# mitenjain/nanopore

Measured on AMD Instinct MI355X. Metric: DP cells/sec (banded pair-HMM realign: forward + backward + posterior per cell), higher is better.
Workload: dtype f32

## Files before the change

### include/nprealign.h

```cpp
#ifndef NPREALIGN_H
#define NPREALIGN_H

#include <stddef.h>
#include <stdint.h>

#ifdef __cplusplus
extern "C" {
#endif

#define NPR_ABI_VERSION 1

#define NPR_OK 0
#define NPR_ERR_INVALID (-1)
#define NPR_ERR_ZERO_PROB (-2)
#define NPR_ERR_CAPACITY (-3)
#define NPR_ERR_MODEL (-4)
#define NPR_ERR_NO_DEVICE (-5)
#define NPR_ERR_HIP (-6)
#define NPR_ERR_BAND_TOO_WIDE (-7)
#define NPR_ERR_NOMEM (-8)
#define NPR_ERR_STATE (-9)

#define NPR_OP_M 0
#define NPR_OP_I 1
// ... 57 lines not shown
#define NPR_OPT_RELEASE_SCRATCH 2
#define NPR_OPT_KERNEL 3
#define NPR_OPT_ARITH 4
#define NPR_OPT_PAIR 5
#define NPR_OPT_NO_TILE 6
#define NPR_OPT_NO_WIDE 7
#define NPR_OPT_TILE_RS 8
#define NPR_OPT_TILE_WAVES 9
#define NPR_OPT_HOST_MEA 13
#define NPR_OPT_MEA_RING_ONLY 14
#define NPR_OPT_MEA_GLOBAL_SORT 15
#define NPR_OPT_EM_GENERIC 17
#define NPR_OPT_MEA_WIDE_OPS 20
#define NPR_OPT_EM_TILE 21
#define NPR_OPT_FINISH_TEXT 22
#define NPR_OPT_COUNT 23
int32_t npr_ctx_option(npr_ctx *ctx, int32_t option, int64_t value);

int32_t npr_set_hmm(npr_ctx *ctx, int32_t slot, const double *T25, const double *E80);

int32_t npr_batch_create(npr_ctx *ctx, const npr_params *params, int64_t n_reads, int64_t n_refs,
                         const uint8_t *ref, const int64_t *ref_off, const int32_t *ref_index,
                         const uint8_t *read, const int64_t *read_off, const int32_t *guide_ops,
                         const int64_t *guide_off, const int32_t *model_slot, npr_batch **out);
int32_t npr_batch_create_at(npr_ctx *ctx, const npr_params *params, int64_t n_reads, int64_t n_refs,
                            const uint8_t *ref, const int64_t *ref_off, const int32_t *ref_index,
                            const uint8_t *read, const int64_t *read_off, const int32_t *guide_ops,
                            const int64_t *guide_off, const int64_t *guide_start, const int32_t *model_slot,
                            npr_batch **out);
int32_t npr_batch_run(npr_batch *b, float *kernel_ms);
int32_t npr_batch_finish(npr_batch *b);
void npr_batch_destroy(npr_batch *b);

int32_t npr_batch_get_stats(const npr_batch *b, npr_batch_stats *st);
int32_t npr_batch_class_stats(const npr_batch *b, int64_t *tasks, int64_t *cells, int32_t cap);
int32_t npr_batch_segment_arith(const npr_batch *b, int64_t *seg_off, int32_t *arith, int64_t cap);
int32_t npr_batch_results(const npr_batch *b, npr_read_result *out );
int32_t npr_batch_ops(const npr_batch *b, int64_t *ops_off, int32_t *ops, int64_t cap_pairs);
int32_t npr_batch_ops_packed(const npr_batch *b, int64_t *ops_off, uint32_t *words, int64_t cap_words);
int32_t npr_batch_pairs(const npr_batch *b, int64_t *pair_off, int32_t *x, int32_t *y, float *p, int64_t cap);
int32_t npr_batch_debug_set_pairs(npr_batch *b, int64_t read, const int32_t *x, const int32_t *y, const float *p, int64_t n, int32_t task_status);

#define NPR_STATS_WORDS 40
int32_t npr_batch_align_stats(npr_batch *b, int32_t *stats );
int32_t npr_align_stats(npr_ctx *ctx, int64_t n_reads, int64_t n_refs, const uint8_t *ref, const int64_t *ref_off,
                        const int32_t *ref_index, const uint8_t *read, const int64_t *read_off, const int32_t *ops,
                        const int64_t *ops_off, const int64_t *start, int32_t *stats );


int32_t npr_kmer_counts(npr_ctx *ctx, int32_t k, int64_t n_seqs, const uint8_t *seq, const int64_t *seq_off,
                        int64_t *counts );
int32_t npr_kmer_counts_groups(npr_ctx *ctx, int32_t k, int64_t n_seqs, const uint8_t *text, const int64_t *seq_begin,
                               const int64_t *seq_end, const int32_t *group, int32_t n_groups,
                               int64_t *counts );
int32_t npr_align_indel_kmers(npr_ctx *ctx, int32_t k, int64_t n_reads, int64_t n_refs, const uint8_t *ref, const int64_t *ref_off,
                              const int32_t *ref_index, const uint8_t *read, const int64_t *read_off, const int32_t *ops,
// ... 92 lines not shown
```

### nanopore_amd/_lib.py

```python
import ctypes as C
import os

import numpy as np

_HERE = os.path.dirname(os.path.abspath(__file__))
LIB_LOADED = False


def want_hw_queues(n=8):
    have = os.environ.get("GPU_MAX_HW_QUEUES")
    if have is None:
        os.environ["GPU_MAX_HW_QUEUES"] = str(n)
    if os.environ.get("NPR_TIMING") or os.environ.get("NPR_JOB_TRACE"):
        import sys
        sys.stderr.write("[npr] GPU_MAX_HW_QUEUES %s%s\n" % (
            "left at the host's %s" % have if have is not None else "set to %d for this process and its children" % n,
            " (the library is already loaded: the runtime may have read it before)" if LIB_LOADED and have is None else ""))


LIB_PATH = os.environ.get("NPR_LIB") or os.path.join(_HERE, "libnprealign.so")

OK = 0
ERR_INVALID, ERR_ZERO_PROB, ERR_CAPACITY, ERR_MODEL, ERR_NO_DEVICE, ERR_HIP, ERR_BAND_TOO_WIDE, ERR_NOMEM, \
    ERR_STATE = -1, -2, -3, -4, -5, -6, -7, -8, -9
OP_M, OP_I, OP_D = 0, 1, 2
BAND_ANCHOR, BAND_FIXED = 0, 1
MODE_REALIGN, MODE_RESCORE_ORIGINAL, MODE_ALL_POSTERIORS, MODE_EXPECTATIONS = 0, 1, 2, 3
OPT_OVERLAP = 1
OPT_RELEASE_SCRATCH = 2
OPTIONS = dict(kernel=3, arith=4, pair=5, no_tile=6, no_wide=7, tile_rs=8, tile_waves=9, host_mea=13, mea_ring_only=14,
               mea_global_sort=15, em_generic=17, mea_wide_ops=20, em_tile=21, finish_text=22)
OPT_FINISH_TEXT = 22
KERNEL_GENERIC, ARITH_CELL, PAIR_NEVER, PAIR_LONG, PAIR_ALL = 1, 1, 1, 2, 3
STATS_WORDS = 40
KMER_MAX_K = 6
KMER_MAX_GROUPS = 64
SAM_COLS = 16
PILEUP_WORDS = 8
MAX_MODELS = 8
E_DEAD = -(1 << 28)


class Params(C.Structure):
    _fields_ = [
        ("band_mode", C.c_int32),
        ("diagonal_expansion", C.c_int32),
# ... 39 lines not shown
    ]


class NprError(RuntimeError):
    def __init__(self, code, where, detail=""):
        self.code = code
        msg = "%s failed: %s (%d)" % (where, strerror(code), code)
        if detail:
            msg += " -- " + detail
        RuntimeError.__init__(self, msg)


EXPORTS = [
    "npr_abi_version", "npr_strerror", "npr_create", "npr_destroy", "npr_last_error", "npr_set_hmm",
    "npr_batch_create", "npr_batch_create_at", "npr_batch_run", "npr_batch_finish", "npr_batch_destroy", "npr_batch_get_stats", "npr_batch_class_stats",
    "npr_batch_results", "npr_batch_ops", "npr_batch_ops_packed", "npr_batch_pairs", "npr_batch_debug_set_pairs", "npr_batch_dense", "npr_batch_rs_forward", "npr_batch_expectations",
    "npr_batch_align_stats", "npr_align_stats", "npr_batch_plan_check", "npr_batch_base_expectations",
    "npr_kmer_counts", "npr_kmer_counts_groups", "npr_align_indel_kmers", "npr_batch_indel_kmers",
    "npr_pileup_create", "npr_pileup_destroy", "npr_pileup_add_batch", "npr_pileup_add", "npr_pileup_counts", "npr_pileup_depth",
    "npr_realign_batch",
    "npr_plan_create", "npr_plan_destroy", "npr_plan_segments", "npr_plan_segment_info",
    "npr_plan_segment_band", "npr_plan_frame_schedule", "npr_plan_stripes", "npr_format_cigars", "npr_format_cigars_packed", "npr_format_sam_records", "npr_chain_hits", "npr_mea_cigar", "npr_rescore", "npr_encode_bases",
    "npr_sam_index", "npr_sam_parse", "npr_sam_guides", "npr_sam_splice", "npr_fasta_index", "npr_fasta_pack", "npr_fastq_index", "npr_names_mark",
    "npr_batch_create_spans", "npr_chain_merge", "npr_ctx_option", "npr_batch_segment_arith",
    "npr_cigar_text_packed", "npr_batch_cigar_text", "npr_sam_splice_text",
]

_lib = None


def load():
# ... 36 lines not shown
    L.npr_batch_finish.argtypes = [vp]
    L.npr_batch_destroy.restype = None
    L.npr_batch_destroy.argtypes = [vp]
    L.npr_batch_get_stats.restype = i32
    L.npr_batch_get_stats.argtypes = [vp, C.POINTER(BatchStats)]
    L.npr_batch_results.restype = i32
    L.npr_batch_results.argtypes = [vp, vp]
    L.npr_batch_ops.restype = i32
    L.npr_batch_ops.argtypes = [vp, vp, vp, i64]
    L.npr_batch_ops_packed.restype = i32
    L.npr_batch_ops_packed.argtypes = [vp, vp, vp, i64]
    L.npr_batch_pairs.restype = i32
    L.npr_batch_pairs.argtypes = [vp, vp, vp, vp, vp, i64]
    L.npr_batch_debug_set_pairs.restype = i32
    L.npr_batch_debug_set_pairs.argtypes = [vp, i64, vp, vp, vp, i64, i32]
    L.npr_batch_expectations.restype = i32
    L.npr_batch_expectations.argtypes = [vp, vp, vp, vp, C.POINTER(C.c_float)]
    L.npr_batch_base_expectations.restype = i32
    L.npr_batch_base_expectations.argtypes = [vp, vp, i64, vp, vp, vp]
    L.npr_batch_plan_check.restype = i64
    L.npr_batch_plan_check.argtypes = [vp, vp]
    L.npr_batch_align_stats.restype = i32
    L.npr_batch_align_stats.argtypes = [vp, vp]
    L.npr_align_stats.restype = i32
    L.npr_align_stats.argtypes = [vp, i64, i64, vp, vp, vp, vp, vp, vp, vp, vp, vp]
    L.npr_kmer_counts.restype = i32
    L.npr_kmer_counts.argtypes = [vp, i32, i64, vp, vp, vp]
    L.npr_kmer_counts_groups.restype = i32
    L.npr_kmer_counts_groups.argtypes = [vp, i32, i64, vp, vp, vp, vp, i32, vp]
    L.npr_align_indel_kmers.restype = i32
# ... 84 lines not shown
```

### nanopore_amd/csrc/npr_api_internal.h

```cpp
#pragma once
#include <hip/hip_runtime.h>

#include <algorithm>
#include <atomic>
#include <chrono>
#include <cmath>
#include <cstdio>
#include <cstdlib>
#include <cstring>
#include <exception>
#include <memory>
#include <mutex>
#include <new>
#include <numeric>
#include <string>
#include <thread>
#include <type_traits>
#include <vector>

#include "npr_device.h"
#include "npr_internal.h"
#include "npr_sched.h"
#include "npr_threads.h"

// ... 246 lines not shown
    int64_t packed_cap = 0;
    bool have_pairs_form = false, have_packed_form = false;
    bool ops_from_guide = false;
    bool rs_staged = false;
    int rs_shift = 0;
    std::vector<int64_t> rs_columns, rs_kept;
    DevBuf<int32_t> d_rs_gy;
    DevBuf<int64_t> d_rs_gx_off;
    std::vector<int64_t> pair_off;
    std::vector<Pair> pairs;
    bool pairs_ready = false;
    std::vector<int64_t> task_dst;
    const uint32_t *dev_ops = nullptr;
    const int64_t *dev_od = nullptr;
    uint64_t dev_ops_epoch = 0;
    std::unique_ptr<char[]> text;
    int64_t text_cap = 0;
    std::vector<int64_t> text_off;
    bool text_ready = false, words_on_device = false;
};

struct npr_pileup {
    npr_ctx *ctx = nullptr;
    std::vector<int64_t> len;
    std::vector<int64_t> base;
    int64_t rows = 0;
    DevBuf<int32_t> tab;
    DevBuf<int32_t> diff;
    DevBuf<int32_t> tile;
    DevBuf<int64_t> dbase;
// ... 99 lines not shown
```

### nanopore_amd/csrc/npr_device.h

```cpp
#pragma once
#include <cstdint>

#include "npr_internal.h"
#include "npr_band.h"

namespace npr {

struct Task {
    int64_t x_off;
    int64_t y_off;
    int64_t band_off;
    int64_t pair_off;
    int32_t lX, lY;
    int32_t D;
    int32_t pair_cap;
    int32_t flags;
    int32_t model;
    int32_t xs, ys;
    int32_t read;
    int32_t cells_pad;
    int64_t ctl_off;
    int64_t tile_off;
    int64_t rowmask_off;
};
// ... 68 lines not shown
int launch_stair(const KernelArgs &a, int R, int grid, void *stream);
int launch_wide(const KernelArgs &a, int R, int NW, int grid, void *stream);
int launch_em_stair(const KernelArgs &a, int R, int grid, void *stream);
size_t em_stair_lds_bytes();
struct MeaArgs {
    const Task *tasks;
    const TaskOut *outs;
    int32_t ntasks, n_reads;
    const int32_t *px, *py;
    const float *pp;
    const int64_t *rx_off;
    const int64_t *ry_off;
    const int64_t *rp_off;
    int32_t *cnt, *start, *colsum;
    int32_t *sx, *sy, *sq, *back;
    int32_t *kx, *ky, *kq, *kback;
    int4 *vrec;
    int32_t *kept;
    const int32_t *np, *poff, *pboff, *lane_read, *lane_piece;
    int32_t *pb, *pbest;
    int32_t n_pieces;
    int32_t *best_who;
    int32_t *read_flag;
    double gap_gamma, match_gamma;
    int32_t ring;
    const int32_t *order;
    const int32_t *read_first, *read_ntasks, *task_of;
    int32_t sort_lds_bytes;
    int32_t sort_threads;
    int32_t any_global_sort;
    const int64_t *cnt_off;
    int32_t ring_only;
    int32_t *ops_tmp;
    const int64_t *ot_off;
    int32_t *n_ops, *chain_len;
    int64_t *chain_mass;
    uint32_t *ops_dense;
    const int64_t *od_off;
    int32_t *max_run;
    uint16_t *ops_dense16;
};
int launch_tile(const KernelArgs &a, int R, int NW, int grid, void *stream, bool flat = false);
size_t tile_lds_bytes(int nw);
// ... 222 lines not shown
```

### nanopore_amd/csrc/npr_finish.cpp

```cpp
#include "npr_api_internal.h"

extern "C" {

}
namespace npr_impl {

int32_t fetch_pairs(npr_batch *b) {
    npr_ctx *ctx = b->ctx;
    if (b->pairs_ready) return NPR_OK;
    StageTimer tm("fetch_pairs");
    const int64_t ntasks = static_cast<int64_t>(b->tasks.size());
    const std::vector<int64_t> &dst = b->task_dst;
    const int32_t *hx = nullptr, *hy = nullptr;
    const float *hp = nullptr;
    const int64_t total = ntasks ? dst[ntasks] : 0;
    if (total) {
        DevBuf<int64_t> d_dst;
        DevBuf<int32_t> d_cx, d_cy;
        DevBuf<float> d_cp;
        hipError_t e;
        if ((e = d_dst.alloc_from(ctx, ntasks + 1)) != hipSuccess || (e = d_cx.alloc_from(ctx, total)) != hipSuccess ||
            (e = d_cy.alloc_from(ctx, total)) != hipSuccess || (e = d_cp.alloc_from(ctx, total)) != hipSuccess)
            return fail(ctx, NPR_ERR_NOMEM, "npr_batch_finish: hipMalloc", e);
        HIP_TRY(ctx, hipMemcpyAsync(d_dst.p, dst.data(), d_dst.bytes(), hipMemcpyHostToDevice, ctx->stream));
// ... 168 lines not shown
        ry[i + 1] = ry[i] + lY;
        rp[i + 1] = rp[i] + np;
        ot[i + 1] = ot[i] + 3 * std::min({np, lX, lY}) + 2;
    }
    const int ring = 8192;
    const int64_t total = rp[n];
    constexpr int64_t kMaxPieces = 64, kLanesWanted = 64 * 5 * 256;
    const int64_t kPiecePairs = std::min<int64_t>(2048, std::max<int64_t>(128, total / kLanesWanted));
    std::vector<int32_t> np(n);
    int64_t n_pieces = 0;
    for (int64_t i = 0; i < n; ++i) np[i] = static_cast<int32_t>(std::min(kMaxPieces, std::max<int64_t>(1, (rp[i + 1] - rp[i] + kPiecePairs - 1) / kPiecePairs))), n_pieces += np[i];
    if (!ctx->mea) ctx->mea = new MeaScratch;
    MeaScratch &m = *ctx->mea;
    hipError_t e;
    const int64_t lds_span = ctx->opt[NPR_OPT_MEA_GLOBAL_SORT] != 0 ? 0 : 16 * 1024;
    int64_t span = 0;
    std::vector<int64_t> cnt_off(n + 1, -1);
    int64_t cnt_total = 0;
    for (int64_t i = 0; i < n; ++i) {
        const int64_t sp = std::max(rx[i + 1] - rx[i], ry[i + 1] - ry[i]);
        if (sp <= lds_span) span = std::max(span, sp);
        else cnt_off[i] = cnt_total, cnt_total += rx[i + 1] - rx[i];
    }
    const bool sort_in_lds = cnt_total == 0;
    const size_t ntask_map = b->task_of.size();
    const size_t n_cnt = sort_in_lds ? 1 : static_cast<size_t>(cnt_total);
    {
        auto al = [](size_t bytes) { return (bytes + 255) & ~size_t(255); };
        const size_t need = al(8 * 5 * (n + 1)) + al(8 * n) + al(8 * (n + 1)) + 2 * al(4 * n_cnt) + al(4 * (ry[n] + 1)) + al(4 * (12 * total + 16)) +
                            al(4 * 6 * n) + al(4 * 2 * ot[n]) + al(4 * (3 * n + ntask_map)) + al(4 * ot[n]) + al(4 * (4 * n_pieces + 4 * n));
        const bool arena_fits = ctx->arena->F && need <= static_cast<size_t>(ctx->arena->cells.load()) * 8;
        bool in_arena = !ctx->overlap && arena_fits;
        for (;;) {
            char *cur = ctx->arena->F;
            if (in_arena && poison_byte() >= 0) {
                HIP_TRY(ctx, hipStreamSynchronize(ctx->stream));
                poison(ctx->arena->F, need);
            }
            auto take = [&](auto &buf, size_t count) -> hipError_t {
                using T = std::remove_pointer_t<decltype(buf.p)>;
                if (!in_arena) return buf.reserve(count);
                buf.borrow(reinterpret_cast<T *>(cur), count);
                cur += al(sizeof(T) * count);
                return hipSuccess;
            };
            if ((e = take(m.off, 5 * (n + 1))) == hipSuccess && (e = take(m.mass, n)) == hipSuccess && (e = take(m.od, n + 1)) == hipSuccess &&
                (e = take(m.cnt, n_cnt)) == hipSuccess && (e = take(m.start, n_cnt)) == hipSuccess && (e = take(m.col, ry[n] + 1)) == hipSuccess &&
                (e = take(m.sorted, 12 * total + 16)) == hipSuccess && (e = take(m.small, 6 * n)) == hipSuccess && (e = take(m.tmp, 2 * ot[n])) == hipSuccess &&
                (e = take(m.map, 3 * n + ntask_map)) == hipSuccess && (e = take(m.dense, ot[n])) == hipSuccess &&
                (e = take(m.pieces, 4 * n_pieces + 4 * n)) == hipSuccess)
                break;
            (void)hipGetLastError();
            if (!in_arena && ctx->overlap && arena_fits) {
                m.off.release(), m.mass.release(), m.od.release(), m.cnt.release(), m.start.release(), m.col.release(), m.sorted.release();
                m.small.release(), m.tmp.release(), m.map.release(), m.dense.release(), m.pieces.release();
                ctx->cache_flush();
                arena_lock.lock();
                if (!(ctx->arena->F && need <= static_cast<size_t>(ctx->arena->cells.load()) * 8)) return 1;
                ++ctx->arena->epoch;
                in_arena = true;
                continue;
            }
            return 1;
// ... 22 lines not shown
    std::copy(cnt_off.begin(), cnt_off.end(), offs.begin() + 4 * (n + 1));
    std::copy(rx.begin(), rx.end(), offs.begin());
    std::copy(ry.begin(), ry.end(), offs.begin() + (n + 1));
    std::copy(rp.begin(), rp.end(), offs.begin() + 2 * (n + 1));
    std::copy(ot.begin(), ot.end(), offs.begin() + 3 * (n + 1));
    HIP_TRY(ctx, hipMemcpyAsync(m.off.p, offs.data(), m.off.bytes(), hipMemcpyHostToDevice, ctx->stream));
    HIP_TRY(ctx, hipMemsetAsync(m.small.p, 0, m.small.bytes(), ctx->stream));
    MeaArgs a{};
    a.tasks = b->d_tasks.p, a.outs = b->d_outs.p, a.ntasks = static_cast<int32_t>(ntasks), a.n_reads = static_cast<int32_t>(n);
    a.px = b->d_px.p, a.py = b->d_py.p, a.pp = b->d_pp.p;
    a.rx_off = m.off.p, a.ry_off = m.off.p + (n + 1), a.rp_off = m.off.p + 2 * (n + 1), a.ot_off = m.off.p + 3 * (n + 1);
    a.cnt = m.cnt.p, a.start = m.start.p, a.colsum = m.col.p;
    a.sx = m.sorted.p, a.sy = m.sorted.p + total + 1, a.sq = m.sorted.p + 2 * (total + 1), a.back = m.sorted.p + 3 * (total + 1);
    a.kx = m.sorted.p + 4 * (total + 1), a.ky = m.sorted.p + 5 * (total + 1), a.kq = m.sorted.p + 6 * (total + 1), a.kback = m.sorted.p + 7 * (total + 1);
    a.vrec = reinterpret_cast<int4 *>(m.sorted.p + ((8 * (total + 1) + 3) & ~int64_t(3)));
    a.best_who = m.small.p, a.read_flag = m.small.p + n, a.n_ops = m.small.p + 2 * n, a.chain_len = m.small.p + 3 * n, a.kept = m.small.p + 4 * n, a.max_run = m.small.p + 5 * n;
    a.chain_mass = m.mass.p;
    a.np = m.pieces.p, a.poff = m.pieces.p + n, a.pboff = m.pieces.p + 2 * n, a.lane_read = m.pieces.p + 3 * n, a.lane_piece = m.pieces.p + 3 * n + n_pieces;
    a.pbest = m.pieces.p + 3 * n + 2 * n_pieces, a.pb = m.pieces.p + 3 * n + 3 * n_pieces, a.n_pieces = static_cast<int32_t>(n_pieces);
    a.gap_gamma = b->params.gap_gamma, a.match_gamma = b->params.match_gamma, a.ring = ring;
    a.ring_only = ctx->opt[NPR_OPT_MEA_RING_ONLY] != 0 ? 1 : 0;
    a.read_first = m.map.p, a.read_ntasks = m.map.p + n, a.task_of = m.map.p + 2 * n, a.order = m.map.p + 2 * n + ntask_map;
    a.sort_lds_bytes = static_cast<int32_t>(4 * span);
    a.sort_threads = ctx->overlap == 1 ? 512 : 0;
    a.any_global_sort = sort_in_lds ? 0 : 1;
    a.cnt_off = m.off.p + 4 * (n + 1);
    a.ops_tmp = m.tmp.p, a.od_off = m.od.p;
    int rc = launch_mea_sort(a, ctx->stream);
    if (rc == 0) rc = launch_mea_chain(a, ctx->stream);
    if (rc != 0) return fail(ctx, NPR_ERR_HIP, "MEA kernel launch", static_cast<hipError_t>(rc));
    std::vector<int32_t> small(6 * n);
    std::vector<int64_t> mass(n);
    HIP_TRY(ctx, hipMemcpyAsync(small.data(), m.small.p, m.small.bytes(), hipMemcpyDeviceToHost, ctx->stream));
    HIP_TRY(ctx, hipMemcpyAsync(mass.data(), m.mass.p, m.mass.bytes(), hipMemcpyDeviceToHost, ctx->stream));
    HIP_TRY(ctx, hipStreamSynchronize(ctx->stream));
    tm.lap("sort + chain + trace");
    const int32_t *flag = small.data() + n, *nops = small.data() + 2 * n, *clen = small.data() + 3 * n;
    int32_t longest = 0;
// ... 60 lines not shown
                failed = 1;
                return;
            }
            const int64_t lo = std::min(nops_all, c * piece), hi = std::min(nops_all, lo + piece);
            if (narrow) {
                const uint16_t *src = reinterpret_cast<const uint16_t *>(pin);
                for (int64_t i = lo; i < hi; ++i) out[i] = src[i];
            } else {
                std::memcpy(out + lo, pin + word * lo, word * static_cast<size_t>(hi - lo));
            }
        });
        if (failed) return fail(ctx, NPR_ERR_HIP, "npr_batch_finish: D2H of the ops", hipGetLastError());
    }
    tm.lap("gather + D2H of the ops");
    if (od[n]) b->dev_ops = m.dense.p, b->dev_od = m.od.p, b->dev_ops_epoch = ctx->arena->epoch;
    return NPR_OK;
}

}
extern "C" {

static int32_t batch_finish_impl(npr_batch *b);

int32_t npr_batch_finish(npr_batch *b) {
    try {
        return batch_finish_impl(b);
    } catch (const std::exception &) {
        return fail(b ? b->ctx : nullptr, NPR_ERR_NOMEM, "npr_batch_finish: out of host memory");
    }
}
// ... 2 lines not shown
    if (!b) return NPR_ERR_INVALID;
    npr_ctx *ctx = b->ctx;
    if (!b->ran) return fail(ctx, NPR_ERR_STATE, "npr_batch_finish before npr_batch_run");
    HIP_TRY(ctx, hipSetDevice(ctx->device));
    StageTimer tm("batch_finish");
    const int64_t ntasks = static_cast<int64_t>(b->tasks.size());
    const int64_t n = b->n_reads;
    std::vector<int64_t> &dst = b->task_dst;
    dst.assign(ntasks + 1, 0);
    if (ntasks) HIP_TRY(ctx, hipMemcpy(b->outs.data(), b->d_outs.p, b->d_outs.bytes(), hipMemcpyDeviceToHost));
    for (int64_t k = 0; k < ntasks; ++k) dst[k + 1] = dst[k] + std::min(b->outs[k].npairs, b->tasks[k].pair_cap);
    b->results.assign(n, npr_read_result{});
    b->pair_off.assign(n + 1, 0);
    b->pairs_ready = false;
    b->text_ready = false, b->words_on_device = false;
    const double LN2 = 0.69314718055994530942;
    for (int64_t i = 0; i < n; ++i) {
        npr_read_result &r = b->results[i];
        r.status = b->read_status[i];
        r.n_segments = b->read_ntasks[i];
        int64_t c = 0;
        if (r.status == NPR_OK)
            for (int32_t s = 0; s < b->read_ntasks[i]; ++s) {
                const int32_t k = b->task_of[b->read_first_task[i] + s];
                const TaskOut &o = b->outs[k];
                if (o.status != NPR_OK && r.status == NPR_OK) r.status = o.status;
                r.cells += b->task_cells[k];
                if (o.tot_m > 0.f) r.loglik += (std::log2(static_cast<double>(o.tot_m)) + o.tot_e) * LN2;
                if (o.btot_m > 0.f) r.loglik_bwd += (std::log2(static_cast<double>(o.btot_m)) + o.btot_e) * LN2;
                c += dst[k + 1] - dst[k];
// ... 1 lines not shown
        r.n_pairs = c;
        b->pair_off[i + 1] = b->pair_off[i] + c;
    }
    tm.lap("task results");
    std::vector<double> dev_score;
    bool have_dev_score = false;
    if (b->params.mode == NPR_MODE_RESCORE_ORIGINAL && n > 0 && ntasks > 0 && b->rs_staged && ctx->opt[NPR_OPT_HOST_MEA] == 0) {
        const int32_t rc = rescore_sum(b, dev_score);
        if (rc < 0) return rc;
        have_dev_score = true;
        tm.lap("device rescore");
    }
    if ((b->params.mode == NPR_MODE_REALIGN || b->params.mode == NPR_MODE_ALL_POSTERIORS) && n > 0 && ntasks > 0 && ctx->opt[NPR_OPT_HOST_MEA] == 0) {
        int64_t scratch = 0;
        for (int64_t i = 0; i < n; ++i) scratch += 8 * (b->ref_len[i] + 1) + 4 * b->read_len[i] + 36 * std::min(b->ref_len[i], b->read_len[i]) + 128;
        scratch += 48 * b->pair_off[n];
        size_t mem_free = 0, mem_total = 0;
        const size_t arena_bytes = ctx->arena->cells.load() * 8;
        if (static_cast<size_t>(scratch) <= arena_bytes ||
            (hipMemGetInfo(&mem_free, &mem_total) == hipSuccess && static_cast<size_t>(scratch) < mem_free / 2)) {
            const int32_t rc = device_mea(b);
            if (rc < 0) return rc;
            if (rc == NPR_OK) {
                tm.lap("device MEA");
                b->finished = true;
                return NPR_OK;
            }
        }
    }
    if (!have_dev_score) {
        const int32_t rc = fetch_pairs(b);
// ... 186 lines not shown
    if (n > tk.pair_cap) return NPR_ERR_CAPACITY;
    HIP_TRY(ctx, hipSetDevice(ctx->device));
    if (n) {
        HIP_TRY(ctx, hipMemcpy(b->d_px.p + tk.pair_off, x, sizeof(int32_t) * n, hipMemcpyHostToDevice));
        HIP_TRY(ctx, hipMemcpy(b->d_py.p + tk.pair_off, y, sizeof(int32_t) * n, hipMemcpyHostToDevice));
        HIP_TRY(ctx, hipMemcpy(b->d_pp.p + tk.pair_off, p, sizeof(float) * n, hipMemcpyHostToDevice));
    }
    TaskOut o;
    HIP_TRY(ctx, hipMemcpy(&o, b->d_outs.p + k, sizeof(TaskOut), hipMemcpyDeviceToHost));
    o.npairs = static_cast<int32_t>(n), o.status = task_status;
    HIP_TRY(ctx, hipMemcpy(b->d_outs.p + k, &o, sizeof(TaskOut), hipMemcpyHostToDevice));
    b->finished = false;
    return NPR_OK;
}


}
```

### nanopore_amd/csrc/npr_mea.hip

```cpp
#include <hip/hip_runtime.h>

#include "npr_device.h"

namespace npr {
namespace {

constexpr int64_t P1 = PROB_ONE;
constexpr int WAVE = 64;
constexpr int SORT_THREADS = 1024;

__device__ __forceinline__ int rdlane(int v, int j) { return __builtin_amdgcn_readlane(v, j); }
__device__ __forceinline__ int64_t rdlane64(int64_t v, int j) {
    const int lo = __builtin_amdgcn_readlane(static_cast<int>(v), j);
    const int hi = __builtin_amdgcn_readlane(static_cast<int>(v >> 32), j);
    return (static_cast<int64_t>(hi) << 32) | static_cast<uint32_t>(lo);
}
__device__ __forceinline__ void wave_sync() {
    __builtin_amdgcn_fence(__ATOMIC_RELEASE, "wavefront");
    __builtin_amdgcn_wave_barrier();
    __builtin_amdgcn_fence(__ATOMIC_ACQUIRE, "wavefront");
}
__device__ __forceinline__ bool beats(int64_t s, int w, int64_t os, int ow) { return s > os || (s == os && w > ow); }

__device__ __forceinline__ int mea_task_pairs(const TaskOut &o, const Task &tk) { return o.status == NPR_OK ? min(max(o.npairs, 0), tk.pair_cap) : 0; }
// ... 56 lines not shown

__global__ void __launch_bounds__(256) k_mea_scatter(MeaArgs a) {
    for (int t = blockIdx.x; t < a.ntasks; t += gridDim.x) {
        const Task &tk = a.tasks[t];
        const int n = mea_task_pairs(a.outs[t], tk);
        const int r = tk.read;
        const int64_t rx = a.cnt_off[r], rp = a.rp_off[r];
        if (rx < 0) continue;
        const int lX = static_cast<int>(a.rx_off[r + 1] - a.rx_off[r]) - 1, lY = static_cast<int>(a.ry_off[r + 1] - a.ry_off[r]);
        for (int i = threadIdx.x; i < n; i += blockDim.x) {
            const int x = a.px[tk.pair_off + i], y = a.py[tk.pair_off + i];
            if (x < 0 || x >= lX || y < 0 || y >= lY || !mea_is_posterior(a.pp[tk.pair_off + i])) continue;
            const int q = static_cast<int>(floor(static_cast<double>(a.pp[tk.pair_off + i]) * static_cast<double>(P1)));
            const int64_t pos = rp + a.start[rx + x] + (atomicSub(a.cnt + rx + x, 1) - 1);
            a.sx[pos] = x, a.sy[pos] = y, a.sq[pos] = q;
        }
    }
}

__global__ void __launch_bounds__(SORT_THREADS) k_mea_sort_lds(MeaArgs a) {
    extern __shared__ int h[];
    __shared__ int wsum[SORT_THREADS / WAVE];
    const int r = a.order[blockIdx.x], tid = threadIdx.x, lane = tid & 63, wv = tid >> 6;
    const int nthreads = static_cast<int>(blockDim.x);
    const int64_t rx = a.rx_off[r], ry = a.ry_off[r], rp = a.rp_off[r];
    const int lX = static_cast<int>(a.rx_off[r + 1] - rx) - 1, lY = static_cast<int>(a.ry_off[r + 1] - ry);
    if (a.rp_off[r + 1] == rp || a.cnt_off[r] >= 0) return;
    const int ft = a.read_first[r], nt = a.read_ntasks[r];
    int bad = 0;
    auto for_pairs = [&](auto f) {
        for (int s = 0; s < nt; ++s) {
            const int t = a.task_of[ft + s];
            const Task &tk = a.tasks[t];
            const int n = mea_task_pairs(a.outs[t], tk);
            for (int i = tid; i < n; i += nthreads) {
                const int x = a.px[tk.pair_off + i], y = a.py[tk.pair_off + i];
                if (x < 0 || x >= lX || y < 0 || y >= lY || !mea_is_posterior(a.pp[tk.pair_off + i])) {
                    bad = 1;
                    continue;
                }
                f(x, y, static_cast<int>(floor(static_cast<double>(a.pp[tk.pair_off + i]) * static_cast<double>(P1))));
            }
        }
    };
    for (int i = tid; i < lY; i += nthreads) h[i] = 0;
    __syncthreads();
    for_pairs([&](int, int y, int q) { atomicAdd(&h[y], q); });
    __syncthreads();
    for (int i = tid; i < lY; i += nthreads) a.colsum[ry + i] = h[i];
    __syncthreads();
    for (int i = tid; i <= lX; i += nthreads) h[i] = 0;
    __syncthreads();
    for_pairs([&](int x, int, int) { atomicAdd(&h[x], 1); });
    __syncthreads();
    int carry = 0;
    for (int base = 0; base <= lX; base += nthreads) {
        const int i = base + tid;
        const int v = i <= lX ? h[i] : 0;
        int sc = v;
        for (int o = 1; o < WAVE; o <<= 1) {
            const int t = __shfl_up(sc, o);
            if (lane >= o) sc += t;
        }
        if (lane == WAVE - 1) wsum[wv] = sc;
        __syncthreads();
        int before = 0, total = 0;
        for (int k = 0; k < nthreads / WAVE; ++k) before += k < wv ? wsum[k] : 0, total += wsum[k];
        if (i <= lX) h[i] = carry + before + sc - v;
        carry += total;
        __syncthreads();
    }
    for_pairs([&](int x, int y, int q) {
        const int64_t pos = rp + atomicAdd(&h[x], 1);
        a.sx[pos] = x, a.sy[pos] = y, a.sq[pos] = q;
    });
    if (bad) a.read_flag[r] = NPR_ERR_INVALID;
}

constexpr int MEA_RETRY = 1;

struct Chunk {
    int valid;
    uint64_t ends;
    uint64_t keep;
    int y, q;
    int64_t w;
    int who;
};
__device__ __forceinline__ Chunk prep_chunk(const MeaArgs &a, int *sx, int *sy, int *sq, int64_t ry, int base, int n, int lane,
// ... 33 lines not shown
    c.who = gfirst + gend - lane;
    if (act) sy[base + c.who] = c.y, sq[base + c.who] = c.q;
    return c;
}

constexpr int WEIGH_CHUNK = 128;
constexpr int WEIGH_RING = 512;
constexpr int WEIGH_HALO = 64;
__device__ __forceinline__ int64_t pair_weight(int q, int rowsum, int colsum, double gap_gamma) {
    const int64_t gap = max(P1 - rowsum, int64_t(0)) + max(P1 - colsum, int64_t(0));
    return q - static_cast<int64_t>(floor(gap_gamma * static_cast<double>(gap)));
}
__global__ void __launch_bounds__(WAVE) k_mea_weigh(MeaArgs a) {
    __shared__ int X[WEIGH_RING], Y[WEIGH_RING], Q[WEIGH_RING], C[WEIGH_RING];
    const int r = a.order[blockIdx.x], lane = threadIdx.x;
    const int64_t rp = a.rp_off[r], ry = a.ry_off[r];
    const int n = a.read_flag[r] ? 0 : static_cast<int>(a.rp_off[r + 1] - rp);
    const int *const sx = a.sx + rp, *const sy = a.sy + rp, *const sq = a.sq + rp;
    const int *const col = a.colsum + ry;
    const int64_t floor_w = static_cast<int64_t>(floor(a.match_gamma * static_cast<double>(P1)));
    constexpr int RM = WEIGH_RING - 1;
    const int nc = (n + WEIGH_CHUNK - 1) / WEIGH_CHUNK;
    int giveup = 0;
    int fx[2], fy[2], fq[2];
    auto fetch = [&](int chunk) {
#pragma unroll
        for (int h = 0; h < 2; ++h) {
            const int j = chunk * WEIGH_CHUNK + h * WAVE + lane;
            const bool ok = j < n;
            fx[h] = ok ? sx[j] : -1, fy[h] = ok ? sy[j] : 0, fq[h] = ok ? sq[j] : 0;
        }
    };
    auto stage = [&](int chunk) {
        int fc[2];
#pragma unroll
        for (int h = 0; h < 2; ++h) fc[h] = fx[h] >= 0 ? col[fy[h]] : 0;
#pragma unroll
        for (int h = 0; h < 2; ++h) {
            const int k = (chunk * WEIGH_CHUNK + h * WAVE + lane) & RM;
            X[k] = fx[h], Y[k] = fy[h], Q[k] = fq[h], C[k] = fc[h];
        }
    };
    for (int k = lane; k < WEIGH_CHUNK; k += WAVE) X[(-WEIGH_CHUNK + k) & RM] = -2;
    if (nc > 0) {
        fetch(0);
        stage(0);
        fetch(1);
    }
    int carry = 0;
    for (int c = 0; c < nc; ++c) {
        stage(c + 1);
// ... 422 lines not shown
```

### nanopore_amd/realign.py

```python
import contextlib
import ctypes as C
import weakref

import numpy as np

from . import _lib
from ._lib import (BAND_ANCHOR, BAND_FIXED, ERR_CAPACITY, ERR_NOMEM, MODE_ALL_POSTERIORS, MODE_EXPECTATIONS, MODE_REALIGN, MODE_RESCORE_ORIGINAL, NprError,
                   Params, ptr)


def make_params(band_mode=BAND_ANCHOR, diagonal_expansion=10, constraint_trim=14, split_threshold=3000,
                fixed_width=0, gap_gamma=0.5, match_gamma=0.0, posterior_threshold=0.01, mode=MODE_REALIGN,
                max_pairs_per_base=0):
    return Params(band_mode, diagonal_expansion, constraint_trim, split_threshold, fixed_width, gap_gamma,
                  match_gamma, posterior_threshold, mode, max_pairs_per_base)


def _csr(seqs):
    lens = np.fromiter((len(s) for s in seqs), dtype=np.int64, count=len(seqs))
    off = np.zeros(len(seqs) + 1, dtype=np.int64)
    np.cumsum(lens, out=off[1:])
    buf = np.empty(int(off[-1]), dtype=np.uint8)
    for i, s in enumerate(seqs):
        if isinstance(s, str):
# ... 112 lines not shown
            raise NprError(int(total), "npr_batch_cigar_text", self.ctx.last_error())
        if buffer is None or buffer.size < max(int(total), 1):
            buffer = np.empty(max(int(total), 1), dtype=np.uint8)
        rc = self._L.npr_batch_cigar_text(self._h, ptr(off), ptr(buffer), int(total))
        if rc < 0:
            raise NprError(int(rc), "npr_batch_cigar_text", self.ctx.last_error())
        return buffer[:int(total)], off

    def debug_set_pairs(self, read, x, y, p, task_status=0):
        x = np.ascontiguousarray(x, np.int32)
        y = np.ascontiguousarray(y, np.int32)
        p = np.ascontiguousarray(p, np.float32)
        rc = self._L.npr_batch_debug_set_pairs(self._h, int(read), ptr(x), ptr(y), ptr(p), len(x), int(task_status))
        if rc != 0:
            raise NprError(rc, "npr_batch_debug_set_pairs")

    def pairs(self):
        off = np.zeros(self.n_reads + 1, dtype=np.int64)
        rc = self._L.npr_batch_pairs(self._h, ptr(off), None, None, None, 0)
        if rc != _lib.OK:
            raise NprError(rc, "npr_batch_pairs")
        k = int(off[-1])
        x = np.zeros(k, dtype=np.int32)
        y = np.zeros(k, dtype=np.int32)
        p = np.zeros(k, dtype=np.float32)
        rc = self._L.npr_batch_pairs(self._h, ptr(off), ptr(x), ptr(y), ptr(p), k)
        if rc != _lib.OK:
            raise NprError(rc, "npr_batch_pairs")
        return off, x, y, p

# ... 548 lines not shown
```

Baseline: 373.1 billion.

## Precompute column sums into sorted pair records and fuse MEA histogram passes

The MEA sort stage now writes each pair's column-sum value into a new sorted array, so the weigh kernel reads it contiguously instead of gathering colsum[y] at random. When an LDS budget option allows, the sort kernel builds the y-column histogram and the x-count histogram in one pass over the pairs rather than two. This adds one extra int per pair of scratch and more LDS per block, and the fused path only runs when the new option is set to a nonzero value. A debug export for reading back the MEA tables is also added.

```diff
diff --git a/include/nprealign.h b/include/nprealign.h
--- a/include/nprealign.h
+++ b/include/nprealign.h
@@ -95,7 +95,8 @@
 #define NPR_OPT_MEA_WIDE_OPS 20
 #define NPR_OPT_EM_TILE 21
 #define NPR_OPT_FINISH_TEXT 22
-#define NPR_OPT_COUNT 23
+#define NPR_OPT_MEA_SORT2_LDS 23
+#define NPR_OPT_COUNT 24
 int32_t npr_ctx_option(npr_ctx *ctx, int32_t option, int64_t value);
 
 int32_t npr_set_hmm(npr_ctx *ctx, int32_t slot, const double *T25, const double *E80);
@@ -121,6 +122,7 @@
 int32_t npr_batch_ops_packed(const npr_batch *b, int64_t *ops_off, uint32_t *words, int64_t cap_words);
 int32_t npr_batch_pairs(const npr_batch *b, int64_t *pair_off, int32_t *x, int32_t *y, float *p, int64_t cap);
 int32_t npr_batch_debug_set_pairs(npr_batch *b, int64_t read, const int32_t *x, const int32_t *y, const float *p, int64_t n, int32_t task_status);
+int32_t npr_batch_debug_mea_tables(const npr_batch *b, int64_t read, int32_t *colsum, int64_t cap_y, int32_t *sorted4, int64_t cap_pairs, int64_t *n_pairs);
 
 #define NPR_STATS_WORDS 40
 int32_t npr_batch_align_stats(npr_batch *b, int32_t *stats );
diff --git a/nanopore_amd/_lib.py b/nanopore_amd/_lib.py
--- a/nanopore_amd/_lib.py
+++ b/nanopore_amd/_lib.py
@@ -29,7 +29,7 @@
 OPT_OVERLAP = 1
 OPT_RELEASE_SCRATCH = 2
 OPTIONS = dict(kernel=3, arith=4, pair=5, no_tile=6, no_wide=7, tile_rs=8, tile_waves=9, host_mea=13, mea_ring_only=14,
-               mea_global_sort=15, em_generic=17, mea_wide_ops=20, em_tile=21, finish_text=22)
+               mea_global_sort=15, em_generic=17, mea_wide_ops=20, em_tile=21, finish_text=22, mea_sort2_lds=23)
 OPT_FINISH_TEXT = 22
 KERNEL_GENERIC, ARITH_CELL, PAIR_NEVER, PAIR_LONG, PAIR_ALL = 1, 1, 1, 2, 3
 STATS_WORDS = 40
@@ -99,7 +99,7 @@
 EXPORTS = [
     "npr_abi_version", "npr_strerror", "npr_create", "npr_destroy", "npr_last_error", "npr_set_hmm",
     "npr_batch_create", "npr_batch_create_at", "npr_batch_run", "npr_batch_finish", "npr_batch_destroy", "npr_batch_get_stats", "npr_batch_class_stats",
-    "npr_batch_results", "npr_batch_ops", "npr_batch_ops_packed", "npr_batch_pairs", "npr_batch_debug_set_pairs", "npr_batch_dense", "npr_batch_rs_forward", "npr_batch_expectations",
+    "npr_batch_results", "npr_batch_ops", "npr_batch_ops_packed", "npr_batch_pairs", "npr_batch_debug_set_pairs", "npr_batch_debug_mea_tables", "npr_batch_dense", "npr_batch_rs_forward", "npr_batch_expectations",
     "npr_batch_align_stats", "npr_align_stats", "npr_batch_plan_check", "npr_batch_base_expectations",
     "npr_kmer_counts", "npr_kmer_counts_groups", "npr_align_indel_kmers", "npr_batch_indel_kmers",
     "npr_pileup_create", "npr_pileup_destroy", "npr_pileup_add_batch", "npr_pileup_add", "npr_pileup_counts", "npr_pileup_depth",
@@ -166,6 +166,8 @@
     L.npr_batch_pairs.argtypes = [vp, vp, vp, vp, vp, i64]
     L.npr_batch_debug_set_pairs.restype = i32
     L.npr_batch_debug_set_pairs.argtypes = [vp, i64, vp, vp, vp, i64, i32]
+    L.npr_batch_debug_mea_tables.restype = i32
+    L.npr_batch_debug_mea_tables.argtypes = [vp, i64, vp, i64, vp, i64, C.POINTER(i64)]
     L.npr_batch_expectations.restype = i32
     L.npr_batch_expectations.argtypes = [vp, vp, vp, vp, C.POINTER(C.c_float)]
     L.npr_batch_base_expectations.restype = i32
diff --git a/nanopore_amd/csrc/npr_api_internal.h b/nanopore_amd/csrc/npr_api_internal.h
--- a/nanopore_amd/csrc/npr_api_internal.h
+++ b/nanopore_amd/csrc/npr_api_internal.h
@@ -284,6 +284,9 @@
     const uint32_t *dev_ops = nullptr;
     const int64_t *dev_od = nullptr;
     uint64_t dev_ops_epoch = 0;
+    const int32_t *dev_col = nullptr, *dev_sorted[4] = {nullptr, nullptr, nullptr, nullptr};
+    const int64_t *dev_mea_off = nullptr;
+    uint64_t mea_epoch = 0;
     std::unique_ptr<char[]> text;
     int64_t text_cap = 0;
     std::vector<int64_t> text_off;
diff --git a/nanopore_amd/csrc/npr_device.h b/nanopore_amd/csrc/npr_device.h
--- a/nanopore_amd/csrc/npr_device.h
+++ b/nanopore_amd/csrc/npr_device.h
@@ -106,6 +106,7 @@
     const int64_t *rp_off;
     int32_t *cnt, *start, *colsum;
     int32_t *sx, *sy, *sq, *back;
+    int32_t *sc;
     int32_t *kx, *ky, *kq, *kback;
     int4 *vrec;
     int32_t *kept;
@@ -119,6 +120,7 @@
     const int32_t *order;
     const int32_t *read_first, *read_ntasks, *task_of;
     int32_t sort_lds_bytes;
+    int32_t sort2_lds_bytes;
     int32_t sort_threads;
     int32_t any_global_sort;
     const int64_t *cnt_off;
diff --git a/nanopore_amd/csrc/npr_finish.cpp b/nanopore_amd/csrc/npr_finish.cpp
--- a/nanopore_amd/csrc/npr_finish.cpp
+++ b/nanopore_amd/csrc/npr_finish.cpp
@@ -206,12 +206,14 @@
     MeaScratch &m = *ctx->mea;
     hipError_t e;
     const int64_t lds_span = ctx->opt[NPR_OPT_MEA_GLOBAL_SORT] != 0 ? 0 : 16 * 1024;
-    int64_t span = 0;
     std::vector<int64_t> cnt_off(n + 1, -1);
     int64_t cnt_total = 0;
+    constexpr int64_t kSortLdsMax = 160 * 1024 - 1024;
+    const int64_t sort2_bytes = std::min(std::max<int64_t>(ctx->opt[NPR_OPT_MEA_SORT2_LDS], 0), kSortLdsMax);
+    int64_t sort_lds = 0;
     for (int64_t i = 0; i < n; ++i) {
-        const int64_t sp = std::max(rx[i + 1] - rx[i], ry[i + 1] - ry[i]);
-        if (sp <= lds_span) span = std::max(span, sp);
+        const int64_t sp = std::max(rx[i + 1] - rx[i], ry[i + 1] - ry[i]), both = 4 * ((rx[i + 1] - rx[i]) + (ry[i + 1] - ry[i]));
+        if (sp <= lds_span) sort_lds = std::max(sort_lds, both <= sort2_bytes ? both : 4 * sp);
         else cnt_off[i] = cnt_total, cnt_total += rx[i + 1] - rx[i];
     }
     const bool sort_in_lds = cnt_total == 0;
@@ -219,7 +221,7 @@
     const size_t n_cnt = sort_in_lds ? 1 : static_cast<size_t>(cnt_total);
     {
         auto al = [](size_t bytes) { return (bytes + 255) & ~size_t(255); };
-        const size_t need = al(8 * 5 * (n + 1)) + al(8 * n) + al(8 * (n + 1)) + 2 * al(4 * n_cnt) + al(4 * (ry[n] + 1)) + al(4 * (12 * total + 16)) +
+        const size_t need = al(8 * 5 * (n + 1)) + al(8 * n) + al(8 * (n + 1)) + 2 * al(4 * n_cnt) + al(4 * (ry[n] + 1)) + al(4 * (13 * total + 16)) +
                             al(4 * 6 * n) + al(4 * 2 * ot[n]) + al(4 * (3 * n + ntask_map)) + al(4 * ot[n]) + al(4 * (4 * n_pieces + 4 * n));
         const bool arena_fits = ctx->arena->F && need <= static_cast<size_t>(ctx->arena->cells.load()) * 8;
         bool in_arena = !ctx->overlap && arena_fits;
@@ -238,7 +240,7 @@
             };
             if ((e = take(m.off, 5 * (n + 1))) == hipSuccess && (e = take(m.mass, n)) == hipSuccess && (e = take(m.od, n + 1)) == hipSuccess &&
                 (e = take(m.cnt, n_cnt)) == hipSuccess && (e = take(m.start, n_cnt)) == hipSuccess && (e = take(m.col, ry[n] + 1)) == hipSuccess &&
-                (e = take(m.sorted, 12 * total + 16)) == hipSuccess && (e = take(m.small, 6 * n)) == hipSuccess && (e = take(m.tmp, 2 * ot[n])) == hipSuccess &&
+                (e = take(m.sorted, 13 * total + 16)) == hipSuccess && (e = take(m.small, 6 * n)) == hipSuccess && (e = take(m.tmp, 2 * ot[n])) == hipSuccess &&
                 (e = take(m.map, 3 * n + ntask_map)) == hipSuccess && (e = take(m.dense, ot[n])) == hipSuccess &&
                 (e = take(m.pieces, 4 * n_pieces + 4 * n)) == hipSuccess)
                 break;
@@ -291,6 +293,7 @@
     a.sx = m.sorted.p, a.sy = m.sorted.p + total + 1, a.sq = m.sorted.p + 2 * (total + 1), a.back = m.sorted.p + 3 * (total + 1);
     a.kx = m.sorted.p + 4 * (total + 1), a.ky = m.sorted.p + 5 * (total + 1), a.kq = m.sorted.p + 6 * (total + 1), a.kback = m.sorted.p + 7 * (total + 1);
     a.vrec = reinterpret_cast<int4 *>(m.sorted.p + ((8 * (total + 1) + 3) & ~int64_t(3)));
+    a.sc = reinterpret_cast<int32_t *>(a.vrec + total);
     a.best_who = m.small.p, a.read_flag = m.small.p + n, a.n_ops = m.small.p + 2 * n, a.chain_len = m.small.p + 3 * n, a.kept = m.small.p + 4 * n, a.max_run = m.small.p + 5 * n;
     a.chain_mass = m.mass.p;
     a.np = m.pieces.p, a.poff = m.pieces.p + n, a.pboff = m.pieces.p + 2 * n, a.lane_read = m.pieces.p + 3 * n, a.lane_piece = m.pieces.p + 3 * n + n_pieces;
@@ -298,7 +301,8 @@
     a.gap_gamma = b->params.gap_gamma, a.match_gamma = b->params.match_gamma, a.ring = ring;
     a.ring_only = ctx->opt[NPR_OPT_MEA_RING_ONLY] != 0 ? 1 : 0;
     a.read_first = m.map.p, a.read_ntasks = m.map.p + n, a.task_of = m.map.p + 2 * n, a.order = m.map.p + 2 * n + ntask_map;
-    a.sort_lds_bytes = static_cast<int32_t>(4 * span);
+    a.sort_lds_bytes = static_cast<int32_t>(sort_lds);
+    a.sort2_lds_bytes = static_cast<int32_t>(sort2_bytes);
     a.sort_threads = ctx->overlap == 1 ? 512 : 0;
     a.any_global_sort = sort_in_lds ? 0 : 1;
     a.cnt_off = m.off.p + 4 * (n + 1);
@@ -389,6 +393,8 @@
     }
     tm.lap("gather + D2H of the ops");
     if (od[n]) b->dev_ops = m.dense.p, b->dev_od = m.od.p, b->dev_ops_epoch = ctx->arena->epoch;
+    b->dev_col = a.colsum, b->dev_sorted[0] = a.sx, b->dev_sorted[1] = a.sy, b->dev_sorted[2] = a.sq, b->dev_sorted[3] = a.sc;
+    b->dev_mea_off = a.rx_off, b->mea_epoch = ctx->arena->epoch;
     return NPR_OK;
 }
 
@@ -421,6 +427,7 @@
     b->pair_off.assign(n + 1, 0);
     b->pairs_ready = false;
     b->text_ready = false, b->words_on_device = false;
+    b->dev_col = nullptr;
     const double LN2 = 0.69314718055994530942;
     for (int64_t i = 0; i < n; ++i) {
         npr_read_result &r = b->results[i];
@@ -452,7 +459,7 @@
     if ((b->params.mode == NPR_MODE_REALIGN || b->params.mode == NPR_MODE_ALL_POSTERIORS) && n > 0 && ntasks > 0 && ctx->opt[NPR_OPT_HOST_MEA] == 0) {
         int64_t scratch = 0;
         for (int64_t i = 0; i < n; ++i) scratch += 8 * (b->ref_len[i] + 1) + 4 * b->read_len[i] + 36 * std::min(b->ref_len[i], b->read_len[i]) + 128;
-        scratch += 48 * b->pair_off[n];
+        scratch += 52 * b->pair_off[n];
         size_t mem_free = 0, mem_total = 0;
         const size_t arena_bytes = ctx->arena->cells.load() * 8;
         if (static_cast<size_t>(scratch) <= arena_bytes ||
@@ -669,5 +676,25 @@
     return NPR_OK;
 }
 
-
-}
+int32_t npr_batch_debug_mea_tables(const npr_batch *b, int64_t read, int32_t *colsum, int64_t cap_y, int32_t *sorted4, int64_t cap_pairs, int64_t *n_pairs) {
+    if (!b || read < 0 || read >= b->n_reads || !n_pairs) return NPR_ERR_INVALID;
+    npr_ctx *ctx = b->ctx;
+    if (!b->finished || !b->dev_col || b->mea_epoch != ctx->arena->epoch)
+        return fail(ctx, NPR_ERR_STATE, "npr_batch_debug_mea_tables: the batch's last finish was not the device MEA stage, or its tables have been overwritten since");
+    HIP_TRY(ctx, hipSetDevice(ctx->device));
+    HIP_TRY(ctx, hipStreamSynchronize(ctx->stream));
+    const int64_t n1 = b->n_reads + 1;
+    int64_t ry[2], rp[2];
+    HIP_TRY(ctx, hipMemcpy(ry, b->dev_mea_off + n1 + read, sizeof(ry), hipMemcpyDeviceToHost));
+    HIP_TRY(ctx, hipMemcpy(rp, b->dev_mea_off + 2 * n1 + read, sizeof(rp), hipMemcpyDeviceToHost));
+    const int64_t lY = ry[1] - ry[0], np = rp[1] - rp[0];
+    *n_pairs = np;
+    if ((colsum && cap_y < lY) || (sorted4 && cap_pairs < np)) return NPR_ERR_CAPACITY;
+    if (colsum && lY) HIP_TRY(ctx, hipMemcpy(colsum, b->dev_col + ry[0], sizeof(int32_t) * lY, hipMemcpyDeviceToHost));
+    if (sorted4 && np)
+        for (int k = 0; k < 4; ++k) HIP_TRY(ctx, hipMemcpy(sorted4 + k * cap_pairs, b->dev_sorted[k] + rp[0], sizeof(int32_t) * np, hipMemcpyDeviceToHost));
+    return NPR_OK;
+}
+
+
+}
diff --git a/nanopore_amd/csrc/npr_mea.hip b/nanopore_amd/csrc/npr_mea.hip
--- a/nanopore_amd/csrc/npr_mea.hip
+++ b/nanopore_amd/csrc/npr_mea.hip
@@ -94,6 +94,7 @@
             const int q = static_cast<int>(floor(static_cast<double>(a.pp[tk.pair_off + i]) * static_cast<double>(P1)));
             const int64_t pos = rp + a.start[rx + x] + (atomicSub(a.cnt + rx + x, 1) - 1);
             a.sx[pos] = x, a.sy[pos] = y, a.sq[pos] = q;
+            a.sc[pos] = a.colsum[a.ry_off[r] + y];
         }
     }
 }
@@ -107,36 +108,47 @@
     const int lX = static_cast<int>(a.rx_off[r + 1] - rx) - 1, lY = static_cast<int>(a.ry_off[r + 1] - ry);
     if (a.rp_off[r + 1] == rp || a.cnt_off[r] >= 0) return;
     const int ft = a.read_first[r], nt = a.read_ntasks[r];
+    const bool two = 4 * (static_cast<int64_t>(lX) + 1 + lY) <= a.sort2_lds_bytes;
+    int *const hy = h, *const hx = two ? h + lY : h;
     int bad = 0;
     auto for_pairs = [&](auto f) {
         for (int s = 0; s < nt; ++s) {
             const int t = a.task_of[ft + s];
             const Task &tk = a.tasks[t];
             const int n = mea_task_pairs(a.outs[t], tk);
-            for (int i = tid; i < n; i += nthreads) {
-                const int x = a.px[tk.pair_off + i], y = a.py[tk.pair_off + i];
-                if (x < 0 || x >= lX || y < 0 || y >= lY || !mea_is_posterior(a.pp[tk.pair_off + i])) {
-                    bad = 1;
-                    continue;
-                }
-                f(x, y, static_cast<int>(floor(static_cast<double>(a.pp[tk.pair_off + i]) * static_cast<double>(P1))));
-            }
+            for (int i = tid; i < n; i += nthreads) f(tk.pair_off + i);
         }
     };
-    for (int i = tid; i < lY; i += nthreads) h[i] = 0;
+    auto x_in = [&](int x) { return static_cast<unsigned>(x) < static_cast<unsigned>(lX); };
+    const int nzero = two ? lY + lX + 1 : lY;
+    for (int i = tid; i < nzero; i += nthreads) h[i] = 0;
     __syncthreads();
-    for_pairs([&](int, int y, int q) { atomicAdd(&h[y], q); });
+    for_pairs([&](int64_t j) {
+        const int x = a.px[j], y = a.py[j];
+        const float p = a.pp[j];
+        if (two && x_in(x)) atomicAdd(&hx[x], 1);
+        if (!x_in(x) || static_cast<unsigned>(y) >= static_cast<unsigned>(lY) || !mea_is_posterior(p)) {
+            bad = 1;
+            return;
+        }
+        atomicAdd(&hy[y], static_cast<int>(floor(static_cast<double>(p) * static_cast<double>(P1))));
+    });
     __syncthreads();
-    for (int i = tid; i < lY; i += nthreads) a.colsum[ry + i] = h[i];
+    for (int i = tid; i < lY; i += nthreads) a.colsum[ry + i] = hy[i];
     __syncthreads();
-    for (int i = tid; i <= lX; i += nthreads) h[i] = 0;
-    __syncthreads();
-    for_pairs([&](int x, int, int) { atomicAdd(&h[x], 1); });
-    __syncthreads();
+    if (!two) {
+        for (int i = tid; i <= lX; i += nthreads) h[i] = 0;
+        __syncthreads();
+        for_pairs([&](int64_t j) {
+            const int x = a.px[j];
+            if (x_in(x)) atomicAdd(&hx[x], 1);
+        });
+        __syncthreads();
+    }
     int carry = 0;
     for (int base = 0; base <= lX; base += nthreads) {
         const int i = base + tid;
-        const int v = i <= lX ? h[i] : 0;
+        const int v = i <= lX ? hx[i] : 0;
         int sc = v;
         for (int o = 1; o < WAVE; o <<= 1) {
             const int t = __shfl_up(sc, o);
@@ -146,13 +158,21 @@
         __syncthreads();
         int before = 0, total = 0;
         for (int k = 0; k < nthreads / WAVE; ++k) before += k < wv ? wsum[k] : 0, total += wsum[k];
-        if (i <= lX) h[i] = carry + before + sc - v;
+        if (i <= lX) hx[i] = carry + before + sc - v;
         carry += total;
         __syncthreads();
     }
-    for_pairs([&](int x, int y, int q) {
-        const int64_t pos = rp + atomicAdd(&h[x], 1);
-        a.sx[pos] = x, a.sy[pos] = y, a.sq[pos] = q;
+    const int *const col = a.colsum + ry;
+    for_pairs([&](int64_t j) {
+        const int x = a.px[j];
+        if (!x_in(x)) return;
+        const int y = a.py[j];
+        const float p = a.pp[j];
+        const bool y_in = static_cast<unsigned>(y) < static_cast<unsigned>(lY);
+        const int64_t pos = rp + atomicAdd(&hx[x], 1);
+        a.sx[pos] = x, a.sy[pos] = y;
+        a.sq[pos] = mea_is_posterior(p) ? static_cast<int>(floor(static_cast<double>(p) * static_cast<double>(P1))) : 0;
+        a.sc[pos] = !y_in ? 0 : two ? hy[y] : col[y];
     });
     if (bad) a.read_flag[r] = NPR_ERR_INVALID;
 }
@@ -216,27 +236,23 @@
 __global__ void __launch_bounds__(WAVE) k_mea_weigh(MeaArgs a) {
     __shared__ int X[WEIGH_RING], Y[WEIGH_RING], Q[WEIGH_RING], C[WEIGH_RING];
     const int r = a.order[blockIdx.x], lane = threadIdx.x;
-    const int64_t rp = a.rp_off[r], ry = a.ry_off[r];
+    const int64_t rp = a.rp_off[r];
     const int n = a.read_flag[r] ? 0 : static_cast<int>(a.rp_off[r + 1] - rp);
-    const int *const sx = a.sx + rp, *const sy = a.sy + rp, *const sq = a.sq + rp;
-    const int *const col = a.colsum + ry;
+    const int *const sx = a.sx + rp, *const sy = a.sy + rp, *const sq = a.sq + rp, *const sc = a.sc + rp;
     const int64_t floor_w = static_cast<int64_t>(floor(a.match_gamma * static_cast<double>(P1)));
     constexpr int RM = WEIGH_RING - 1;
     const int nc = (n + WEIGH_CHUNK - 1) / WEIGH_CHUNK;
     int giveup = 0;
-    int fx[2], fy[2], fq[2];
+    int fx[2], fy[2], fq[2], fc[2];
     auto fetch = [&](int chunk) {
 #pragma unroll
         for (int h = 0; h < 2; ++h) {
             const int j = chunk * WEIGH_CHUNK + h * WAVE + lane;
             const bool ok = j < n;
-            fx[h] = ok ? sx[j] : -1, fy[h] = ok ? sy[j] : 0, fq[h] = ok ? sq[j] : 0;
+            fx[h] = ok ? sx[j] : -1, fy[h] = ok ? sy[j] : 0, fq[h] = ok ? sq[j] : 0, fc[h] = ok ? sc[j] : 0;
         }
     };
     auto stage = [&](int chunk) {
-        int fc[2];
-#pragma unroll
-        for (int h = 0; h < 2; ++h) fc[h] = fx[h] >= 0 ? col[fy[h]] : 0;
 #pragma unroll
         for (int h = 0; h < 2; ++h) {
             const int k = (chunk * WEIGH_CHUNK + h * WAVE + lane) & RM;
diff --git a/nanopore_amd/realign.py b/nanopore_amd/realign.py
--- a/nanopore_amd/realign.py
+++ b/nanopore_amd/realign.py
@@ -150,6 +150,18 @@
         rc = self._L.npr_batch_debug_set_pairs(self._h, int(read), ptr(x), ptr(y), ptr(p), len(x), int(task_status))
         if rc != 0:
             raise NprError(rc, "npr_batch_debug_set_pairs")
+
+    def debug_mea_tables(self, read, n_y):
+        n = C.c_int64(0)
+        rc = self._L.npr_batch_debug_mea_tables(self._h, int(read), None, 0, None, 0, C.byref(n))
+        if rc != _lib.OK:
+            raise NprError(rc, "npr_batch_debug_mea_tables", self.ctx.last_error())
+        colsum = np.zeros(int(n_y), dtype=np.int32)
+        rows = np.zeros((4, max(n.value, 1)), dtype=np.int32)
+        rc = self._L.npr_batch_debug_mea_tables(self._h, int(read), ptr(colsum), len(colsum), ptr(rows), rows.shape[1], C.byref(n))
+        if rc != _lib.OK:
+            raise NprError(rc, "npr_batch_debug_mea_tables", self.ctx.last_error())
+        return colsum, rows[:, :n.value]
 
     def pairs(self):
         off = np.zeros(self.n_reads + 1, dtype=np.int64)
```

Result: faster. 379.0 billion, median of 3 (+1.6%).
